# myshell-ai/OpenVoice

Measured on NVIDIA H100. Metric: audio_seconds_per_second, higher is better.
Workload: dtype f32 (3xFP16 split-precision tensor-core convs with fp32 accumulation, fp32 FFMA elsewhere)

## Files before the change

include/ovc.h:

```cpp
#ifndef OVC_B200_H
#define OVC_B200_H

#include <stddef.h>
#include <stdint.h>

#ifdef __cplusplus
extern "C" {
#endif

#define OVC_ABI_VERSION 12

#if defined(__GNUC__)
#define OVC_API __attribute__((visibility("default")))
#else
#define OVC_API
#endif

enum {
  OVC_OK = 0,
  OVC_ERR_INVALID = -1,
  OVC_ERR_CUDA = -2,
  OVC_ERR_STATE = -3,
  OVC_ERR_MISSING = -4,
  OVC_ERR_NOMEM = -5
};

typedef struct ovc_ctx ovc_ctx;

typedef struct ovc_hparams {
  int32_t spec_channels;
  int32_t inter_channels;
  int32_t hidden_channels;
  int32_t gin_channels;
// ... 92 lines not shown

OVC_API int ovc_tts_encode_state(ovc_ctx* ctx, float* stats, int32_t* cum, float* g, void* stream);

OVC_API int ovc_tts_encode_state_rows(ovc_ctx* ctx, const int64_t* dst_row, int N, int Tp, float* stats, int32_t* cum,
                                      float* g, int64_t* y_lengths, void* stream);
OVC_API int ovc_tts_state_rows(ovc_ctx* ctx, const float* stats, const int32_t* cum, const float* g, const int64_t* y_lengths,
                               int B, int T, const int64_t* dst_row, int N, int Tp, float* d_stats, int32_t* d_cum,
                               float* d_g, int64_t* d_y_lengths, void* stream);

OVC_API int ovc_tts_decode_windows(ovc_ctx* ctx, const float* stats, const int32_t* cum, const float* g,
                                   const int64_t* y_lengths, int N, int T, const int64_t* row, const int64_t* frame0,
                                   const int64_t* len, int W, int Wmax, const uint64_t* seed, const int64_t* stream,
                                   const float* noise_scale, float* o, float* z_p, void* cuda_stream);

OVC_API int ovc_set_precision(ovc_ctx* ctx, int mode);

#define OVC_OPT_TTS_SIMPLE 2
#define OVC_OPT_GRAPH 3
#define OVC_OPT_PDL 5
#define OVC_OPT_BRANCHES 7
#define OVC_OPT_PAIR 8
#define OVC_OPT_PAIR_OCC 9
#define OVC_OPT_STAGED_EPI 10
OVC_API int ovc_set_option(ovc_ctx* ctx, int key, int value);

OVC_API int ovc_last_launch_count(const ovc_ctx* ctx);

OVC_API int ovc_graph_replays(const ovc_ctx* ctx);

OVC_API int ovc_profile_enable(ovc_ctx* ctx, int enable);
OVC_API int ovc_profile_read(ovc_ctx* ctx, double* ms, int64_t* launches, double* flops, double* bytes);
OVC_API int ovc_profile_detail(ovc_ctx* ctx, int max, char* names, double* ms, double* flops, double* bytes,
                               int* family);

OVC_API int ovc_debug_enable(ovc_ctx* ctx, int enable);
OVC_API int ovc_debug_fetch(ovc_ctx* ctx, const char* name, float* host_out, size_t max_floats,
                    int64_t* shape4 );

#ifdef __cplusplus
}
#endif
#endif
```

openvoice_b200/_native.py:

```python
from __future__ import annotations

import ctypes as C
import os
from typing import Dict, Iterable, Optional, Tuple

_HERE = os.path.dirname(os.path.abspath(__file__))
LIB_PATH = os.path.join(_HERE, "libovc_b200.so")

ABI_VERSION = 12
EXPORTS = (
    "ovc_abi_version", "ovc_last_error", "ovc_create", "ovc_destroy", "ovc_load_tensor",
    "ovc_finalize_weights", "ovc_workspace_floats", "ovc_voice_conversion", "ovc_last_launch_count",
    "ovc_profile_enable", "ovc_profile_read", "ovc_profile_detail", "ovc_debug_enable", "ovc_debug_fetch",
    "ovc_spectrogram", "ovc_convert_waveform", "ovc_set_precision", "ovc_reference_encoder",
    "ovc_tts_info", "ovc_tts_encode", "ovc_tts_decode", "ovc_set_option", "ovc_graph_replays",
    "ovc_reference_encoder_ragged", "ovc_resample", "ovc_resample_span", "ovc_voice_conversion_items",
    "ovc_convert_waveform_items", "ovc_tts_encode_items", "ovc_tts_decode_items", "ovc_philox_normals",
    "ovc_tts_encode_state", "ovc_tts_decode_windows", "ovc_spectrogram_ring", "ovc_splice",
    "ovc_tts_encode_state_rows", "ovc_tts_state_rows",
)

STREAM_OPEN = 2 ** 63 - 1
SPLICE_PCM16 = 1


class OvcHParams(C.Structure):
    _fields_ = [
        ("spec_channels", C.c_int32), ("inter_channels", C.c_int32), ("hidden_channels", C.c_int32),
        ("gin_channels", C.c_int32), ("resblock", C.c_int32), ("n_resblock_kernels", C.c_int32),
        ("resblock_kernel_sizes", C.c_int32 * 4), ("resblock_dilations", (C.c_int32 * 3) * 4),
        ("n_upsamples", C.c_int32), ("upsample_rates", C.c_int32 * 4),
        ("upsample_kernel_sizes", C.c_int32 * 4), ("upsample_initial_channel", C.c_int32),
# ... 208 lines not shown
        used, ignored = [], []
        for k, v in sd.items():
            a = v.detach().cpu().float().contiguous().numpy() if hasattr(v, "detach") else np.ascontiguousarray(v, dtype=np.float32)
            if a.ndim == 0 or a.ndim > 4:
                ignored.append(k)
                continue
            shape = (C.c_int64 * a.ndim)(*a.shape)
            rc = self.lib.ovc_load_tensor(self.handle, k.encode(), a.ctypes.data_as(C.c_void_p), shape, a.ndim)
            _check(self.lib, rc, f"ovc_load_tensor({k})")
            (ignored if rc == 1 else used).append(k)
        self.finalized = False
        return used, ignored

    def finalize(self):
        _check(self.lib, self.lib.ovc_finalize_weights(self.handle), "ovc_finalize_weights")
        self.finalized = True

    def set_precision(self, mode: str):
        m = PRECISIONS[mode]
        _check(self.lib, self.lib.ovc_set_precision(self.handle, m), "ovc_set_precision")
        self.precision = mode

    def set_option(self, key: str, value: int):
        k = {"tts_simple": 2, "graph": 3, "pdl": 5, "branches": 7, "pair": 8, "pair_occ": 9, "staged_epi": 10}[key]
        _check(self.lib, self.lib.ovc_set_option(self.handle, k, int(value)), "ovc_set_option")

    def voice_conversion(self, spec, lengths, g_src, g_tgt, noise=None, tau: float = 0.3, seed: int = 0,
                         ragged: bool = False, latents: bool = True, stream=None, items: Optional[dict] = None, out=None):
        import torch
        assert spec.is_cuda and spec.dtype == torch.float32 and spec.is_contiguous()
        assert lengths.is_cuda and lengths.dtype == torch.int64 and lengths.is_contiguous()
        B, S, T = spec.shape
        gs = g_src.reshape(B, -1).contiguous().float()
        gt = g_tgt.reshape(B, -1).contiguous().float()
        if noise is not None:
            noise = noise.contiguous().float()
            assert tuple(noise.shape) == (B, self.hp.inter_channels, T)
        hop = self.hp.hop_length
        if out is not None:
            assert out.is_cuda and out.dtype == torch.float32 and out.is_contiguous() and out.numel() == B * hop * T
            o = out.view(B, 1, hop * T)
        else:
            o = torch.empty(B, 1, hop * T, device=spec.device, dtype=torch.float32)
        lat = None
        if latents:
            lat = tuple(torch.empty(B, self.hp.inter_channels, T, device=spec.device, dtype=torch.float32)
                        for _ in range(3))
# ... 332 lines not shown
```

openvoice_b200/csrc/ovc_lib.cu:

```cuda
#include <cuda_runtime.h>

#include <algorithm>
#include <cmath>
#include <cstdarg>
#include <cstdio>
#include <cstdlib>
#include <cstring>
#include <map>
#include <string>
#include <vector>

#include "../../include/ovc.h"
#include "ovc_convpack.h"
#include "ovc_small.cuh"
#include "ovc_tcconv.cuh"
#include "ovc_tts.cuh"
#include "ovc_refenc.cuh"
#include "ovc_resample.cuh"
#include "ovc_splice.h"
#include "ovc_variants.h"

namespace ovc {

static thread_local std::string g_err;
// ... 66 lines not shown
};

struct ConvLayer {
  int variant = -1;
  int rows = 0;
  int row_tiles = 0;
  int cin = 0;
  int n_chunks = 0;
  size_t w_off = 0;
  size_t b_off = 0;
  int K = 1;
  int cout = 0;
  int out_mul = 1;
};

struct TcLayer : TcGeom {
  size_t w_off = 0;
  size_t b_off = 0;
};

struct WNLayers {
  std::vector<ConvLayer> in, rs;
  std::vector<TcLayer> tc_in, tc_rs;
};

struct Fp32Dense { size_t w = 0, b = 0; int Cin = 0, K = 0, N = 0; bool fast = false; ConvLayer cl; };
struct DdsLayers {
  size_t sep_w[3] = {0}, sep_b[3] = {0}, n1g[3] = {0}, n1b[3] = {0}, n2g[3] = {0}, n2b[3] = {0};
  Fp32Dense c1x1[3];
};
struct TtsLayers {
  bool ready = false;
  int n_vocab = 0, n_speakers = 0, H = 0, C = 0, Fc = 0, heads = 0, n_layers = 0, window = 0, D = 0;
  size_t emb = 0, emb_g = 0;
  std::vector<TcLayer> qkv, o;
  std::vector<Fp32Dense> ffn1, ffn2;
  std::vector<size_t> relk, relv, ln1g, ln1b, ln2g, ln2b;
  TcLayer proj;
  Fp32Dense dp_c1, dp_c2, sdp_pre, sdp_proj;
  size_t dp_n1g = 0, dp_n1b = 0, dp_n2g = 0, dp_n2b = 0, dp_pw = 0, dp_pb = 0, dp_cw = 0, dp_cb = 0, sdp_cw = 0, sdp_cb = 0,
         ea = 0;
  DdsLayers dds[4];
  size_t cf_pre_w[4] = {0}, cf_pre_b[4] = {0}, cf_pw[4] = {0}, cf_pb[4] = {0};
};

struct DebugBuf {
// ... 15 lines not shown

  float* d_w = nullptr;
  size_t w_floats = 0;
  std::vector<float> h_w;

  ConvLayer enc_pre, enc_pre16, enc_proj;
  WNLayers enc_wn;
  ConvLayer flow_pre[4], flow_post[4];
  WNLayers flow_wn[4];
  ConvLayer dec_pre, dec_ups[4];
  ConvLayer rb_c1[12][3], rb_c2[12][3];
  TcLayer tc_c1[12][3], tc_c2[12][3], tc_ups[4], tc_pre;
  float* d_tcw = nullptr;
  std::vector<float> h_tcw;
  int precision = 0;
  bool tts_simple = false;
  bool use_graph = true;
  int use_pdl = 2;
  bool use_branches = true;
  int par_frames = 512;
  bool use_pair = true;
  bool use_pair_occ = true;
  bool use_staged_epi = true;
  bool pair_occ2_ok[TCN_N_OCC2] = {};
  cudaStream_t br_stream[2] = {nullptr, nullptr};
  cudaEvent_t br_ev[4] = {nullptr, nullptr, nullptr, nullptr};
  size_t post_w_off = 0;
  size_t cond_w_off = 0, cond_b_off = 0;
  int* d_cond_wrow = nullptr;
  int* d_cond_sel = nullptr;
  int cond_rows_out = 0;
  int cond_off_enc = 0, cond_off_fsrc = 0, cond_off_ftgt = 0, cond_off_dec = 0;
  int cond_off_enc_tc = 0, cond_off_fsrc_tc = 0, cond_off_ftgt_tc = 0;

  float2* d_tw = nullptr;
  float* d_win = nullptr;

  bool has_refenc = false;
  size_t re_conv_w[6] = {0}, re_conv_b[6] = {0}, re_wih = 0, re_whh = 0, re_bih = 0, re_bhh = 0, re_pw = 0, re_pb = 0,
         re_lng = 0, re_lnb = 0;
  int re_gru_in = 0;
  float* d_re = nullptr;
  size_t re_floats = 0;

  std::map<std::pair<int64_t, int64_t>, double*> rs_banks;
  bool rs_smem_opt_in = false;
// ... 177 lines not shown
  const int H = 192;
  *out = WNLayers();
  for (int i = 0; i < n_layers; ++i) {
    HostTensor w, r;
    const HostTensor* rb;
    const std::string prs = prefix + ".res_skip_layers." + std::to_string(i);
    const int rows = (i < n_layers - 1) ? 2 * H : H;
    TRY(conv_weight(c, prefix + ".in_layers." + std::to_string(i), {2 * H, H, 5}, &w));
    TRY(conv_weight(c, prs, {rows, H, 1}, &r));
    TRY(tensor(c, prs + ".bias", {rows}, &rb));
    out->in.push_back(pack_conv(
        c, V_WN_IN, 2 * H, H,
        [&](int p, int ci, int k) { return w.data[((size_t)paired_row(p, H) * H + ci) * 5 + k]; },
        [&](int) { return 0.f; }, 0, 5, 2 * H));
    out->rs.push_back(pack_conv(
        c, V_WN_RS, rows, H, [&](int p, int ci, int) { return r.data[(size_t)p * H + ci]; },
        [&](int p) { return rb->data[p]; }, rows, 1, rows));
    out->tc_in.push_back(pack_tc(
        c, 2 * H, H, 5, 1, [&](int p, int ci, int k) { return w.data[((size_t)paired_row32(p, H) * H + ci) * 5 + k]; },
        [&](int) { return 0.f; }));
    out->tc_rs.push_back(pack_tc(
        c, rows, H, 1, 1, [&](int p, int ci, int) { return r.data[(size_t)p * H + ci]; },
        [&](int p) { return rb->data[p]; }));
  }
  return OVC_OK;
}

#include "ovc_tts_pack.inc"

static int finalize(ovc_ctx* c) {
  const ovc_hparams& hp = c->hp;
  const int H = 192, S = hp.spec_channels, G = hp.gin_channels;
  drop_graphs(c);
  c->h_w.clear();
  c->h_tcw.clear();

  {
    const HostTensor *w, *b, *pw, *pb;
    TRY(tensor(c, "enc_q.pre.weight", {H, S, 1}, &w));
    TRY(tensor(c, "enc_q.pre.bias", {H}, &b));
    c->enc_pre = pack_conv(c, V_ENC_PRE, H, S, [&](int p, int ci, int) { return w->data[(size_t)p * S + ci]; },
                           [&](int p) { return b->data[p]; }, H, 1, H);
    c->enc_pre16 = c->enc_pre;
    c->enc_pre16.variant = V_FLOW_PRE;
    TRY(pack_wn(c, "enc_q.enc", 16, &c->enc_wn));
    TRY(tensor(c, "enc_q.proj.weight", {2 * H, H, 1}, &pw));
// ... 148 lines not shown
      TRY(tensor(c, e.key, e.shape, &t));
      *e.off = append(c->h_w, t->data);
    }
    c->has_refenc = true;
  }
  c->tts = TtsLayers();
  if (find(c, "enc_p.emb.weight")) TRY(pack_tts(c));
  ON_DEVICE(c);
  if (c->d_w) { cudaFree(c->d_w); c->d_w = nullptr; }
  c->w_floats = c->h_w.size();
  CK(cudaMalloc(&c->d_w, c->w_floats * sizeof(float)));
  CK(cudaMemcpy(c->d_w, c->h_w.data(), c->w_floats * sizeof(float), cudaMemcpyHostToDevice));
  if (c->d_tcw) { cudaFree(c->d_tcw); c->d_tcw = nullptr; }
  CK(cudaMalloc(&c->d_tcw, c->h_tcw.size() * sizeof(float)));
  CK(cudaMemcpy(c->d_tcw, c->h_tcw.data(), c->h_tcw.size() * sizeof(float), cudaMemcpyHostToDevice));
  c->h_tcw.clear();
  c->h_tcw.shrink_to_fit();
  for (int TN : {128, 64, 32})
    for (bool staged : {false, true}) {
      const TcKernel k = tc_conv_kernel(TN, staged), p = tc_pair_kernel(TN, TcPairOcc(), staged);
      CK(cudaFuncSetAttribute(k.fn, cudaFuncAttributeMaxDynamicSharedMemorySize, (int)k.smem));
      CK(cudaFuncSetAttribute(p.fn, cudaFuncAttributeMaxDynamicSharedMemorySize, (int)p.smem));
    }
  for (int i = 0; i < TCN_N_OCC2; ++i) {
    const TcKernel k = tc_pair_kernel(kTcPairOcc2[i].C, kTcPairOcc2[i].o);
    CK(cudaFuncSetAttribute(k.fn, cudaFuncAttributeMaxDynamicSharedMemorySize, (int)k.smem));
    int blocks = 0;
    CK(cudaOccupancyMaxActiveBlocksPerMultiprocessor(&blocks, k.fn, k.threads, k.smem));
    c->pair_occ2_ok[i] = blocks >= 2;
    if (blocks < 2)
      fprintf(stderr, "ovc: the C = %d conv-pair kernel with %d operand buffer(s) fits %d CTA(s) per SM, not 2; its pairs run "
              "one CTA per SM\n", kTcPairOcc2[i].C, kTcPairOcc2[i].o.nabuf, blocks);
  }
  if (c->d_cond_wrow) cudaFree(c->d_cond_wrow);
  if (c->d_cond_sel) cudaFree(c->d_cond_sel);
  CK(cudaMalloc(&c->d_cond_wrow, wrow.size() * sizeof(int)));
  CK(cudaMalloc(&c->d_cond_sel, sel.size() * sizeof(int)));
  CK(cudaMemcpy(c->d_cond_wrow, wrow.data(), wrow.size() * sizeof(int), cudaMemcpyHostToDevice));
  CK(cudaMemcpy(c->d_cond_sel, sel.data(), sel.size() * sizeof(int), cudaMemcpyHostToDevice));
  if (!c->d_tw) {
    std::vector<float2> tw(STFT_N);
    std::vector<float> win(STFT_N);
    const double PI = 3.14159265358979323846;
    for (int m = 0; m < STFT_N; ++m) {
      tw[m] = make_float2((float)std::cos(2.0 * PI * m / STFT_N), (float)(-std::sin(2.0 * PI * m / STFT_N)));
      win[m] = (float)(0.5 - 0.5 * std::cos(2.0 * PI * m / STFT_N));
// ... 109 lines not shown
static int prof_begin(Run& r) {
  ovc_ctx* c = r.c;
  if (!c->prof) return OVC_OK;
  if (c->ev_used + 2 > c->ev.size()) {
    const size_t old = c->ev.size();
    c->ev.resize(old + 512);
    for (size_t i = old; i < c->ev.size(); ++i) CK(cudaEventCreate(&c->ev[i]));
  }
  CK(cudaEventRecord(c->ev[c->ev_used], r.st));
  return OVC_OK;
}
static int prof_end(Run& r, int variant, int family, double flops, double bytes, int tag = 0) {
  ovc_ctx* c = r.c;
  if (!c->prof) return OVC_OK;
  CK(cudaEventRecord(c->ev[c->ev_used + 1], r.st));
  c->ev_used += 2;
  c->ev_flops.push_back(flops);
  c->ev_bytes.push_back(bytes);
  c->ev_variant.push_back(variant);
  c->ev_family.push_back(family);
  c->ev_tag.push_back(tag);
  return OVC_OK;
}
enum { V_TCPAIR128 = -14, V_TCPAIR64 = -12, V_TCPAIR32 = -13, V_TC128 = -1, V_TC64 = -2, V_TC32 = -3, V_TRANSPOSE = -4, V_TTS_DENSE = -5, V_TTS_LN = -6, V_TTS_SCORES = -7,
       V_TTS_ATTN = -8, V_TTS_DW = -9, V_TTS_SPLINE = -10, V_TTS_MISC = -11 };
static const char* variant_name(int v) {
  if (v >= 0) return kInfo[v].name;
  switch (v) {
    case V_TCPAIR128: return "PAIR_N128";
    case V_TCPAIR64: return "PAIR_N64";
    case V_TCPAIR32: return "PAIR_N32";
    case V_TC128: return "TC3_N128";
    case V_TC64: return "TC3_N64";
    case V_TC32: return "TC3_N32";
    case V_TTS_DENSE: return "TTS_DENSE32";
    case V_TTS_LN: return "TTS_LAYERNORM";
    case V_TTS_SCORES: return "TTS_SCORES";
    case V_TTS_ATTN: return "TTS_ATTN_OUT";
    case V_TTS_DW: return "TTS_DWCONV";
    case V_TTS_SPLINE: return "TTS_SPLINE";
    case V_TTS_MISC: return "TTS_MISC";
    default: return "TRANSPOSE";
  }
}

struct TcExtra {
  int epi = 0;
  const float* bias = nullptr;
  long long bias_bs = 0;
  float* s = nullptr;
  int split = 0, first = 0;
// ... 98 lines not shown
  const int n = (int)wn.in.size();
  for (int i = 0; i < n; ++i) {
    ConvArgs a{};
    a.x = x; a.x_bs = bs; a.x_pitch = P;
    a.bias = cond + (size_t)i * 384; a.bias_bs = cond_bs;
    a.y = acts; a.y_bs = bs; a.y_pitch = P;
    a.lens_in = r.lens; a.lens_out = r.lens; a.mul_in = 1; a.mul_out = 1;
    a.slope = 1.f;
    TRY(launch(r, wn.in[i], a, T));
    ConvArgs b{};
    b.x = acts; b.x_bs = bs; b.x_pitch = P;
    b.bias = r.c->d_w + wn.rs[i].b_off; b.bias_bs = 0;
    b.y = x; b.y_bs = bs; b.y_pitch = P;
    b.s = skip; b.s_bs = bs; b.s_pitch = P;
    b.lens_in = r.lens; b.lens_out = r.lens; b.mul_in = 1; b.mul_out = 1;
    b.slope = 1.f;
    b.split = (i < n - 1) ? 192 : 0;
    b.flags = (i == 0) ? F_FIRST : 0;
    TRY(launch(r, wn.rs[i], b, T));
  }
  return OVC_OK;
}

static int run_wn_tc(Run& r, const WNLayers& wn, float* x, float* skip, float* acts, float* x_cl, float* skip_cl,
                     const float* cond_tc, int cond_bs) {
  const int P = r.P, T = r.Tmax;
  const int n = (int)wn.tc_in.size();
  TRY(launch_transpose(r, x, x_cl, 192, P));
  for (int i = 0; i < n; ++i) {
    TcExtra g;
    g.epi = 1; g.bias = cond_tc + (size_t)i * 384; g.bias_bs = cond_bs; g.y_ld = 192; g.use_lens_frames = true;
    TRY(launch_tc(r, wn.tc_in[i], x_cl, acts, nullptr, T, 1, 1.f, 1.f, 0, 0, g));
    TcExtra q;
    q.epi = 2; q.s = skip_cl; q.split = (i < n - 1) ? 192 : 0; q.first = (i == 0); q.y_ld = 192; q.use_lens_frames = true;
    TRY(launch_tc(r, wn.tc_rs[i], acts, x_cl, nullptr, T, 1, 1.f, 1.f, 0, 0, q));
  }
  TRY(launch_transpose(r, skip_cl, skip, P, 192));
  return OVC_OK;
}

static int run_flow(Run& r, const WsLayout& W, float* ws, bool reverse, const float* cond_all) {
  ovc_ctx* c = r.c;
  const int P = r.P, T = r.Tmax;
  const long long bs = 192LL * P;
  float* z = ws + W.z;
  float* x = ws + W.x;
  float* skip = ws + W.skip;
  float* acts = ws + W.acts;
  const int sect = reverse ? c->cond_off_ftgt : c->cond_off_fsrc;
  for (int step = 0; step < 4; ++step) {
    const int f = reverse ? 3 - step : step;
// ... 89 lines not shown
  }
  const cudaError_t ie = cudaGraphInstantiate(&e->exec, graph, 0);
  cudaGraphDestroy(graph);
  if (ie != cudaSuccess) {
    cudaGetLastError();
    e->exec = nullptr;
    e->seen = -1000000;
    return body(st);
  }
  e->launches = c->launches;
  CK(cudaGraphLaunch(e->exec, st));
  c->graph_replays++;
  return OVC_OK;
}

static int set_call_params(ovc_ctx* c, uint64_t seed, float tau, const ItemParams& items, cudaStream_t st) {
  if (!c->d_callp) CK(cudaMalloc(&c->d_callp, sizeof(CallParams)));
  set_call_params_kernel<<<1, 1, 0, st>>>(c->d_callp, seed, tau, items);
  CK(cudaGetLastError());
  return OVC_OK;
}
static uintptr_t option_bits(const ovc_ctx* c) {
  return (uintptr_t)c->precision | ((uintptr_t)c->use_pdl << 15) | ((uintptr_t)c->use_branches << 14) | ((uintptr_t)c->use_pair << 17) |
         ((uintptr_t)c->use_pair_occ << 18) | ((uintptr_t)c->use_staged_epi << 19);
}

static int ensure_ws(ovc_ctx* c, const WsLayout& W, int B, int Tmax, cudaStream_t st) {
  if (W.total <= c->ws_floats) return OVC_OK;
  CK(cudaStreamSynchronize(st));
  drop_graphs(c);
  if (c->d_ws) CK(cudaFree(c->d_ws));
  c->d_ws = nullptr;
  c->ws_floats = 0;
  cudaError_t e = cudaMalloc(&c->d_ws, W.total * sizeof(float));
  if (e != cudaSuccess) {
    cudaGetLastError();
    return fail(OVC_ERR_NOMEM, "workspace of %.2f GB for B=%d Tmax=%d does not fit: %s", W.total * 4e-9, B, Tmax,
                cudaGetErrorString(e));
  }
  c->ws_floats = W.total;
  return OVC_OK;
}

static int copy_latent_out(Run& r, const WsLayout& W, float* ws, float* dst) {
  if (!dst) return OVC_OK;
  dim3 grid((r.Tmax + 255) / 256, 192, r.B);
  copy_latent_kernel<<<grid, 256, 0, r.st>>>(ws + W.z, W.P, dst, r.Tmax, 192, r.lens);
// ... 728 lines not shown
  return OVC_OK;
}

int ovc_set_precision(ovc_ctx* c, int mode) {
  if (!c) return fail(OVC_ERR_INVALID, "null context");
  if (mode < 0 || mode > 2) return fail(OVC_ERR_INVALID, "precision mode must be 0 (fp32 FFMA), 1 (3xFP16 tensor cores) or 2 (single-pass fp16)");
  c->precision = mode;
  return OVC_OK;
}

int ovc_set_option(ovc_ctx* c, int key, int value) {
  if (!c) return fail(OVC_ERR_INVALID, "null context");
  switch (key) {
    case OVC_OPT_TTS_SIMPLE: c->tts_simple = value != 0; return OVC_OK;
    case OVC_OPT_GRAPH: c->use_graph = value != 0; return OVC_OK;
    case OVC_OPT_PDL:
      if (value < 0 || value > 2) return fail(OVC_ERR_INVALID, "pdl must be 0, 1 or 2");
      c->use_pdl = value;
      return OVC_OK;
    case OVC_OPT_BRANCHES: c->use_branches = value != 0; return OVC_OK;
    case OVC_OPT_PAIR: c->use_pair = value != 0; return OVC_OK;
    case OVC_OPT_PAIR_OCC: c->use_pair_occ = value != 0; return OVC_OK;
    case OVC_OPT_STAGED_EPI: c->use_staged_epi = value != 0; return OVC_OK;
    default: return fail(OVC_ERR_INVALID, "unknown option %d", key);
  }
}

int ovc_last_launch_count(const ovc_ctx* c) { return c ? c->launches : 0; }

int ovc_graph_replays(const ovc_ctx* c) { return c ? c->graph_replays : 0; }

int ovc_profile_enable(ovc_ctx* c, int enable) {
  if (!c) return fail(OVC_ERR_INVALID, "null context");
  c->prof = enable != 0;
  c->ev_used = 0;
  c->ev_flops.clear();
  c->ev_bytes.clear();
  c->ev_variant.clear();
  c->ev_family.clear();
  c->ev_tag.clear();
  return OVC_OK;
}

int ovc_profile_read(ovc_ctx* c, double* ms, int64_t* launches, double* flops, double* bytes) {
  if (!c) return fail(OVC_ERR_INVALID, "null context");
  double tms = 0, tf = 0, tb = 0;
// ... 9 lines not shown
  }
  if (ms) *ms = tms;
  if (launches) *launches = n;
  if (flops) *flops = tf;
  if (bytes) *bytes = tb;
  c->ev_used = 0;
  c->ev_flops.clear();
  c->ev_bytes.clear();
  c->ev_variant.clear();
  c->ev_family.clear();
  c->ev_tag.clear();
  return OVC_OK;
}

int ovc_profile_detail(ovc_ctx* c, int max, char* names , double* ms, double* flops, double* bytes, int* family) {
  if (!c) return fail(OVC_ERR_INVALID, "null context");
  int n = 0;
  for (size_t i = 0; i + 1 < c->ev_used && n < max; i += 2, ++n) {
    float m = 0;
    CK(cudaEventElapsedTime(&m, c->ev[i], c->ev[i + 1]));
    if (names) {
      const int tag = c->ev_tag[i / 2], v = c->ev_variant[i / 2];
      if (tag && v == V_TCPAIR128) snprintf(names + 16 * n, 16, "T128Pk%dd%d", (tag >> 8) & 255, tag & 255);
      else if (tag && (v == V_TCPAIR64 || v == V_TCPAIR32)) snprintf(names + 16 * n, 16, "P%dk%dd%d", tag >> 16, (tag >> 8) & 255, tag & 255);
      else if (tag) snprintf(names + 16 * n, 16, "T%dc%dk%dd%d", v == V_TC128 ? 128 : v == V_TC64 ? 64 : 32, tag >> 16, (tag >> 8) & 255, tag & 255);
      else { strncpy(names + 16 * n, variant_name(v), 15); names[16 * n + 15] = 0; }
    }
    if (ms) ms[n] = m;
    if (flops) flops[n] = c->ev_flops[i / 2];
    if (bytes) bytes[n] = c->ev_bytes[i / 2];
    if (family) family[n] = c->ev_family[i / 2];
  }
  return n;
}

int ovc_debug_enable(ovc_ctx* c, int enable) {
  if (!c) return fail(OVC_ERR_INVALID, "null context");
  c->debug = enable != 0;
  return OVC_OK;
}

int ovc_debug_fetch(ovc_ctx* c, const char* name, float* host_out, size_t max_floats, int64_t* shape4) {
  if (!c || !name) return fail(OVC_ERR_INVALID, "null argument");
  auto it = c->taps.find(name);
  if (it == c->taps.end()) return fail(OVC_ERR_INVALID, "no debug tap named '%s' (enable debug and run a call first)", name);
  const DebugBuf& d = it->second;
// ... 13 lines not shown
```

openvoice_b200/csrc/ovc_tcconv.cuh:

```cuda
#pragma once
#include "ovc_conv.cuh"
#include "ovc_tc.cuh"
#include "ovc_tcpack.h"

namespace ovc {

struct TcConvArgs {
  const float* x; long long x_bs;
  const uint16_t* w;
  const float* bias; long long bias_bs;
  float* y; long long y_bs; int y_ld;
  const float* r;
  float* s; long long s_bs;
  int epi;
  int split; int first;
  const long long* lens; int tmax; int mul;
  const long long* lens_x; int has_lens_x;
  int Cin; int Ntot; int K; int DIL;
  float slope; float scale; int accumulate;
  int passes;
  const uint16_t* w2; const float* bias2;
};

__device__ __forceinline__ void pdl_launch_dependents() { asm volatile("griddepcontrol.launch_dependents;" ::: "memory"); }
// ... 92 lines not shown
__device__ __forceinline__ void tc_epilogue(const TcConvArgs& a, const float (&d)[TN], int b, int t0, int n0, int lim, int row_a) {
  const bool two = a.passes == 3;
  tc_epilogue_v<TN>(a, [&](int j) { return tc_result<TN>(d, two, j); }, b, t0, n0, lim, row_a);
}
__device__ __forceinline__ TcConvArgs tc_pair_epilogue_args(const TcConvArgs& a, int TN) {
  TcConvArgs e = a;
  e.y_ld = TN; e.r = a.x; e.bias = a.bias2; e.bias_bs = 0; e.epi = 0;
  return e;
}

template <int TN>
__device__ __forceinline__ void tc_mma_step(float (&d)[TN], uint64_t a_hi, uint64_t a_lo, uint64_t b, bool three, bool first) {
  float (&lo)[TN / 2] = *reinterpret_cast<float(*)[TN / 2]>(&d[TN / 2]);
  float (&hi)[TN / 2] = *reinterpret_cast<float(*)[TN / 2]>(&d[0]);
  tc::Wgmma<TN>::mma(hi, a_hi, b, first ? 0 : 1);
  if (three) {
    tc::Wgmma<TN>::mma(lo, a_hi, b + TN, first ? 0 : 1);
    tc::Wgmma<TN>::mma(lo, a_lo, b, 1);
  }
}

constexpr int TCN_THREADS = 384;
constexpr int TCN_NCT = 96;

template <int TN, bool PAIR, int OCC = 1, int NAB = 2, bool STAGED = false>
struct TcnCfg {
  static_assert(!PAIR || TN == 32 || TN == 64 || TN == 128, "conv pairs: C = 32, 64 or 128");
  static_assert(OCC == 1 || (PAIR && TN <= 64), "two CTAs per SM: C = 32 / 64 pairs");
  static_assert(!STAGED || (TN == 128 && OCC == 1), "staged epilogue: TN = 128, one CTA per SM");
  static constexpr int THREADS = STAGED ? TCN_THREADS + 128 : TCN_THREADS;
  static constexpr int KCH = 32, NKC = KCH / 8;
  static constexpr int ROWS = 194;
  static constexpr int ROWS2 = TCN_ROWS2;
  static constexpr int NABUF = NAB;
  static constexpr int RING = PAIR ? tc_pair_ring(TN, OCC, NAB) : tc_ring_slots(TN, PAIR);
  static constexpr int SLOT_BYTES = 2 * 2 * TN * 16;
  static constexpr int A_BUF_BYTES = 2 * NKC * ROWS * 16;
  static constexpr int A2_BYTES = PAIR ? 2 * (TN / 8) * ROWS2 * 16 : 0;
  static constexpr int STAGE_BYTES = STAGED ? (TN / 2) * 256 * 4 : 0;
  static_assert(!STAGED || !PAIR || STAGE_BYTES <= A2_BYTES, "a pair's staging tile lies in its conv-2 operand");
  static constexpr int SBUF_BYTES = STAGED && !PAIR ? STAGE_BYTES : 0;
  static constexpr size_t SMEM_BYTES = 1024 + NABUF * A_BUF_BYTES + A2_BYTES + RING * SLOT_BYTES + SBUF_BYTES;
  static_assert(!PAIR || SMEM_BYTES == tc_pair_smem(TN, NABUF, RING), "tc_pair_smem");
  static_assert(SMEM_BYTES <= (OCC == 1 ? 232448 : TCN_SMEM_OCC2), "shared memory budget");
  static_assert((2 * NABUF + 2 * RING + 2) * 8 <= 1024, "barrier area");
  static constexpr int PROD_REGS = OCC == 1 && !STAGED ? 56 : 32, MMA_REGS = STAGED ? 184 : OCC == 1 ? 224 : 104;
// ... 287 lines not shown
}
inline bool tc_stage_pays(int K, int passes) { return passes * K >= 15; }
inline TcKernel tc_conv_kernel(int TN, bool staged) {
  if (TN == 128) return staged ? tc_kernel<128, false, 1, 2, true>() : tc_kernel<128, false>();
  if (TN == 64) return tc_kernel<64, false>();
  if (TN == 32) return tc_kernel<32, false>();
  return {};
}
inline TcKernel tc_pair_kernel(int C, TcPairOcc o, bool staged = false) {
  if (o.occ == 1 && o.nabuf == 2) {
    if (C == 128) return staged ? tc_kernel<128, true, 1, 2, true>() : tc_kernel<128, true>();
    if (C == 64) return tc_kernel<64, true>();
    if (C == 32) return tc_kernel<32, true>();
  } else if (o.occ == 2) {
    if (C == 32 && o.nabuf == 2) return tc_kernel<32, true, 2, 2>();
    if (C == 32 && o.nabuf == 1) return tc_kernel<32, true, 2, 1>();
    if (C == 64 && o.nabuf == 1) return tc_kernel<64, true, 2, 1>();
  }
  return {};
}
constexpr int TCN_N_OCC2 = 3;
constexpr struct { int C; TcPairOcc o; } kTcPairOcc2[TCN_N_OCC2] = {{32, {2, 2}}, {32, {2, 1}}, {64, {2, 1}}};

template <int C>
__global__ void __launch_bounds__(256) conv_post_cl_kernel(const float* __restrict__ x, long long x_bs,
                                                           const float* __restrict__ w, float* __restrict__ y,
                                                           long long y_bs, int y_len, const long long* lens, int tmax,
                                                           int mul) {
  constexpr int TB = 256, ROWS = TB + 6, LD = ROWS + 3;
  __shared__ float ws[7][C];
  __shared__ float xs[C][LD];
  for (int i = threadIdx.x; i < C * 7; i += blockDim.x) ws[i % 7][i / 7] = w[i];
  const int b = blockIdx.y;
  const int lim = (lens ? (int)min((long long)tmax, lens[b]) : tmax) * mul;
  const int t0 = blockIdx.x * TB;
  const float* xb = x + (size_t)b * x_bs;
  for (int idx = threadIdx.x; idx < ROWS * (C / 4); idx += blockDim.x) {
    const int row = idx / (C / 4), q = idx % (C / 4);
    const int tt = t0 - 3 + row;
    float4 v = make_float4(0.f, 0.f, 0.f, 0.f);
    if (tt >= 0 && tt < lim) v = *reinterpret_cast<const float4*>(xb + (size_t)tt * C + 4 * q);
    xs[4 * q + 0][row] = v.x > 0.f ? v.x : 0.01f * v.x;
    xs[4 * q + 1][row] = v.y > 0.f ? v.y : 0.01f * v.y;
    xs[4 * q + 2][row] = v.z > 0.f ? v.z : 0.01f * v.z;
    xs[4 * q + 3][row] = v.w > 0.f ? v.w : 0.01f * v.w;
  }
// ... 34 lines not shown
```

openvoice_b200/csrc/ovc_tcpack.h:

```cpp
#pragma once
#include <cuda_fp16.h>
#include <stddef.h>
#include <stdint.h>

#include <algorithm>

namespace ovc {

constexpr int TCN_HMAX = 25;
constexpr int TCN_ROWS2 = 146;

constexpr int tc_ring_slots(int TN, bool pair) {
  return pair ? (TN == 32 ? 44 : TN == 64 ? 24 : 12) : (TN == 32 ? 22 : 12);
}

struct TcGeom {
  int Cin = 0, Ntot = 0, K = 0, DIL = 1, TN = 0;
};

inline int tc_tile_n(int Ntot, int Cin, int K, int DIL) {
  if (Ntot <= 0 || Cin <= 0 || K <= 0 || DIL <= 0) return 0;
  if (Ntot % 32 || Cin % 32 || (K - 1) / 2 * DIL > TCN_HMAX) return 0;
  return Ntot % 128 == 0 ? 128 : (Ntot % 64 == 0 ? 64 : 32);
}
// ... 33 lines not shown
}

template <class RAW>
inline float tc_ups_weight(RAW raw, int s, int kk, int cout, int row, int ci, int tap) {
  const int pad = (kk - s) / 2;
  const int ph = row / cout, co = row % cout;
  const int kidx = s * (1 - tap) + ph + pad;
  return (kidx >= 0 && kidx < kk) ? raw(ci, co, kidx) : 0.f;
}

inline bool tc_pair_fits(const TcGeom& T1, const TcGeom& T2) {
  if (!(T1.TN == 32 || T1.TN == 64)) return false;
  const int ring = tc_ring_slots(T1.TN, true);
  return T1.Ntot == T1.TN && T1.Cin == T1.TN && T2.Ntot == T1.TN && T2.Cin == T1.TN && T2.TN == T1.TN && T2.K == T1.K &&
         T2.DIL == 1 && (T1.K - 1) / 2 * T1.DIL <= TCN_HMAX && 2 * (T1.Cin / 16) * T1.K <= ring && T1.K <= 5;
}

inline bool tc_pair_fuses(const TcGeom& T1, const TcGeom& T2) {
  if (!(T1.TN == 32 || T1.TN == 64 || T1.TN == 128)) return false;
  return T1.Ntot == T1.TN && T1.Cin == T1.TN && T2.Ntot == T1.TN && T2.Cin == T1.TN && T2.TN == T1.TN && T2.K == T1.K &&
         T2.DIL == 1 && (T1.K - 1) / 2 * T1.DIL <= TCN_HMAX && 128 + 2 * ((T2.K - 1) / 2) <= TCN_ROWS2;
}

struct TcGrid {
  int n_tt = 0, total = 0, grid_x = 0, ncol = 0;
};
inline TcGrid tc_grid(int t_len, int B, int Ntot, int TN, int sm_count, int grid_div) {
  TcGrid g;
  g.n_tt = (t_len + 127) / 128;
  g.total = g.n_tt * B;
  g.ncol = Ntot / TN;
  const int per_col = std::max(1, sm_count / g.ncol / std::max(1, grid_div));
  g.grid_x = std::min(g.total, per_col);
  return g;
}
inline TcGrid tc_pair_grid(int t_len, int B, int K, int sm_count, int occ = 1) {
  TcGrid g;
  const int R = 128 - (K - 1);
  g.n_tt = (t_len + R - 1) / R;
  g.total = g.n_tt * B;
  g.ncol = 1;
  g.grid_x = std::min(g.total, occ * sm_count);
  return g;
}

constexpr size_t tc_pair_smem(int TN, int nabuf, int ring) {
  return 1024 + (size_t)nabuf * 2 * 4 * 194 * 16 + (size_t)2 * (TN / 8) * TCN_ROWS2 * 16 + (size_t)ring * 2 * 2 * TN * 16;
}
constexpr size_t TCN_SMEM_OCC2 = (233472 - 2 * 1024) / 2;
constexpr int tc_pair_ring(int TN, int occ, int nabuf) {
  return occ == 1 ? tc_ring_slots(TN, true) : (int)((TCN_SMEM_OCC2 - tc_pair_smem(TN, nabuf, 0)) / (2 * 2 * TN * 16));
}

struct TcPairOcc {
  int occ = 1, nabuf = 2;
};
// ... 12 lines not shown
```

Measured before the change: 2411.

## Fuse WaveNet in-conv, gated activation and res/skip conv into one kernel

```diff
diff --git a/include/ovc.h b/include/ovc.h
--- a/include/ovc.h
+++ b/include/ovc.h
@@ -8,7 +8,7 @@
 extern "C" {
 #endif
 
-#define OVC_ABI_VERSION 12
+#define OVC_ABI_VERSION 13
 
 #if defined(__GNUC__)
 #define OVC_API __attribute__((visibility("default")))
@@ -147,6 +147,7 @@
 #define OVC_OPT_PAIR 8
 #define OVC_OPT_PAIR_OCC 9
 #define OVC_OPT_STAGED_EPI 10
+#define OVC_OPT_WN_FUSE 11
 OVC_API int ovc_set_option(ovc_ctx* ctx, int key, int value);
 
 OVC_API int ovc_last_launch_count(const ovc_ctx* ctx);
diff --git a/openvoice_b200/_native.py b/openvoice_b200/_native.py
--- a/openvoice_b200/_native.py
+++ b/openvoice_b200/_native.py
@@ -7,7 +7,7 @@
 _HERE = os.path.dirname(os.path.abspath(__file__))
 LIB_PATH = os.path.join(_HERE, "libovc_b200.so")
 
-ABI_VERSION = 12
+ABI_VERSION = 13
 EXPORTS = (
     "ovc_abi_version", "ovc_last_error", "ovc_create", "ovc_destroy", "ovc_load_tensor",
     "ovc_finalize_weights", "ovc_workspace_floats", "ovc_voice_conversion", "ovc_last_launch_count",
@@ -262,7 +262,8 @@
         self.precision = mode
 
     def set_option(self, key: str, value: int):
-        k = {"tts_simple": 2, "graph": 3, "pdl": 5, "branches": 7, "pair": 8, "pair_occ": 9, "staged_epi": 10}[key]
+        k = {"tts_simple": 2, "graph": 3, "pdl": 5, "branches": 7, "pair": 8, "pair_occ": 9, "staged_epi": 10,
+             "wn_fuse": 11}[key]
         _check(self.lib, self.lib.ovc_set_option(self.handle, k, int(value)), "ovc_set_option")
 
     def voice_conversion(self, spec, lengths, g_src, g_tgt, noise=None, tau: float = 0.3, seed: int = 0,
diff --git a/openvoice_b200/csrc/ovc_lib.cu b/openvoice_b200/csrc/ovc_lib.cu
--- a/openvoice_b200/csrc/ovc_lib.cu
+++ b/openvoice_b200/csrc/ovc_lib.cu
@@ -112,6 +112,7 @@
 struct WNLayers {
   std::vector<ConvLayer> in, rs;
   std::vector<TcLayer> tc_in, tc_rs;
+  std::vector<TcLayer> tc_rsf;
 };
 
 struct Fp32Dense { size_t w = 0, b = 0; int Cin = 0, K = 0, N = 0; bool fast = false; ConvLayer cl; };
@@ -173,6 +174,7 @@
   bool use_pair = true;
   bool use_pair_occ = true;
   bool use_staged_epi = true;
+  bool use_wn_fuse = true;
   bool pair_occ2_ok[TCN_N_OCC2] = {};
   cudaStream_t br_stream[2] = {nullptr, nullptr};
   cudaEvent_t br_ev[4] = {nullptr, nullptr, nullptr, nullptr};
@@ -396,6 +398,14 @@
     out->tc_rs.push_back(pack_tc(
         c, rows, H, 1, 1, [&](int p, int ci, int) { return r.data[(size_t)p * H + ci]; },
         [&](int p) { return rb->data[p]; }));
+    const int rows_f = tc_wn_rs_rows_packed(rows);
+    if (rows_f == rows) {
+      out->tc_rsf.push_back(out->tc_rs.back());
+    } else {
+      out->tc_rsf.push_back(pack_tc(
+          c, rows_f, H, 1, 1, [&](int p, int ci, int) { return p < rows ? r.data[(size_t)p * H + ci] : 0.f; },
+          [&](int p) { return p < rows ? rb->data[p] : 0.f; }));
+    }
   }
   return OVC_OK;
 }
@@ -590,6 +600,7 @@
       CK(cudaFuncSetAttribute(k.fn, cudaFuncAttributeMaxDynamicSharedMemorySize, (int)k.smem));
       CK(cudaFuncSetAttribute(p.fn, cudaFuncAttributeMaxDynamicSharedMemorySize, (int)p.smem));
     }
+  CK(cudaFuncSetAttribute(tcwn_kernel, cudaFuncAttributeMaxDynamicSharedMemorySize, (int)TcWnCfg::SMEM_BYTES));
   for (int i = 0; i < TCN_N_OCC2; ++i) {
     const TcKernel k = tc_pair_kernel(kTcPairOcc2[i].C, kTcPairOcc2[i].o);
     CK(cudaFuncSetAttribute(k.fn, cudaFuncAttributeMaxDynamicSharedMemorySize, (int)k.smem));
@@ -745,11 +756,12 @@
   c->ev_tag.push_back(tag);
   return OVC_OK;
 }
-enum { V_TCPAIR128 = -14, V_TCPAIR64 = -12, V_TCPAIR32 = -13, V_TC128 = -1, V_TC64 = -2, V_TC32 = -3, V_TRANSPOSE = -4, V_TTS_DENSE = -5, V_TTS_LN = -6, V_TTS_SCORES = -7,
+enum { V_TCWN = -15, V_TCPAIR128 = -14, V_TCPAIR64 = -12, V_TCPAIR32 = -13, V_TC128 = -1, V_TC64 = -2, V_TC32 = -3, V_TRANSPOSE = -4, V_TTS_DENSE = -5, V_TTS_LN = -6, V_TTS_SCORES = -7,
        V_TTS_ATTN = -8, V_TTS_DW = -9, V_TTS_SPLINE = -10, V_TTS_MISC = -11 };
 static const char* variant_name(int v) {
   if (v >= 0) return kInfo[v].name;
   switch (v) {
+    case V_TCWN: return "WN_FUSED";
     case V_TCPAIR128: return "PAIR_N128";
     case V_TCPAIR64: return "PAIR_N64";
     case V_TCPAIR32: return "PAIR_N32";
@@ -894,11 +906,49 @@
   return OVC_OK;
 }
 
+static int launch_wn_layer(Run& r, const TcLayer& Tin, const TcLayer& Trs, const float* x_in, float* x_out, float* skip,
+                           const float* cond, int cond_bs, int split, int first) {
+  TcWnArgs w{};
+  TcConvArgs& a = w.g;
+  a.x = x_in; a.x_bs = 192LL * r.P;
+  a.w = reinterpret_cast<const uint16_t*>(r.c->d_tcw + Tin.w_off);
+  a.bias = cond; a.bias_bs = cond_bs;
+  a.w2 = reinterpret_cast<const uint16_t*>(r.c->d_tcw + Trs.w_off); a.bias2 = r.c->d_tcw + Trs.b_off;
+  a.lens = r.lens; a.tmax = r.Tmax; a.mul = 1;
+  a.Cin = Tin.Cin; a.Ntot = Tin.Ntot; a.K = Tin.K; a.DIL = Tin.DIL;
+  a.slope = 1.f; a.scale = 1.f;
+  a.passes = r.c->precision == 2 ? 1 : 3;
+  w.x_out = x_out; w.s = skip; w.split = split; w.first = first; w.rs_n = split + 192;
+  const TcGrid g = tc_wn_grid(r.Tmax, r.B, r.c->sm_count);
+  TRY(prof_begin(r));
+  CK(launch_ex(tcwn_kernel, dim3((unsigned)g.grid_x, 1, 1), TCN_THREADS, TcWnCfg::SMEM_BYTES, r.st, r.c->use_pdl != 0, w,
+               g.n_tt, g.total));
+  CK(cudaGetLastError());
+  r.c->launches++;
+  const double units = (double)r.B * r.Tmax;
+  TRY(prof_end(r, V_TCWN, 0, 2.0 * 192 * (384.0 * Tin.K + w.rs_n) * units, 4.0 * 192 * (2 + 2 + (first ? 0 : 1)) * units,
+               (Tin.Cin << 16) | (Tin.K << 8) | Tin.DIL));
+  return OVC_OK;
+}
+
 static int run_wn_tc(Run& r, const WNLayers& wn, float* x, float* skip, float* acts, float* x_cl, float* skip_cl,
                      const float* cond_tc, int cond_bs) {
   const int P = r.P, T = r.Tmax;
   const int n = (int)wn.tc_in.size();
   TRY(launch_transpose(r, x, x_cl, 192, P));
+  bool fuse = r.c->use_wn_fuse;
+  for (int i = 0; i < n; ++i) fuse = fuse && tc_wn_fuses(wn.tc_in[i], wn.tc_rs[i], r.c->precision == 2 ? 1 : 3);
+  if (fuse) {
+    float* xa = x_cl;
+    float* xb = acts;
+    for (int i = 0; i < n; ++i) {
+      TRY(launch_wn_layer(r, wn.tc_in[i], wn.tc_rsf[i], xa, xb, skip_cl, cond_tc + (size_t)i * 384, cond_bs,
+                          (i < n - 1) ? 192 : 0, i == 0));
+      std::swap(xa, xb);
+    }
+    TRY(launch_transpose(r, skip_cl, skip, P, 192));
+    return OVC_OK;
+  }
   for (int i = 0; i < n; ++i) {
     TcExtra g;
     g.epi = 1; g.bias = cond_tc + (size_t)i * 384; g.bias_bs = cond_bs; g.y_ld = 192; g.use_lens_frames = true;
@@ -1034,7 +1084,8 @@
 }
 static uintptr_t option_bits(const ovc_ctx* c) {
   return (uintptr_t)c->precision | ((uintptr_t)c->use_pdl << 15) | ((uintptr_t)c->use_branches << 14) | ((uintptr_t)c->use_pair << 17) |
-         ((uintptr_t)c->use_pair_occ << 18) | ((uintptr_t)c->use_staged_epi << 19);
+         ((uintptr_t)c->use_pair_occ << 18) | ((uintptr_t)c->use_staged_epi << 19) |
+         ((uintptr_t)c->use_wn_fuse << 20);
 }
 
 static int ensure_ws(ovc_ctx* c, const WsLayout& W, int B, int Tmax, cudaStream_t st) {
@@ -1809,6 +1860,7 @@
     case OVC_OPT_PAIR: c->use_pair = value != 0; return OVC_OK;
     case OVC_OPT_PAIR_OCC: c->use_pair_occ = value != 0; return OVC_OK;
     case OVC_OPT_STAGED_EPI: c->use_staged_epi = value != 0; return OVC_OK;
+    case OVC_OPT_WN_FUSE: c->use_wn_fuse = value != 0; return OVC_OK;
     default: return fail(OVC_ERR_INVALID, "unknown option %d", key);
   }
 }
@@ -1864,6 +1916,7 @@
     if (names) {
       const int tag = c->ev_tag[i / 2], v = c->ev_variant[i / 2];
       if (tag && v == V_TCPAIR128) snprintf(names + 16 * n, 16, "T128Pk%dd%d", (tag >> 8) & 255, tag & 255);
+      else if (tag && v == V_TCWN) snprintf(names + 16 * n, 16, "WNFc%dk%d", tag >> 16, (tag >> 8) & 255);
       else if (tag && (v == V_TCPAIR64 || v == V_TCPAIR32)) snprintf(names + 16 * n, 16, "P%dk%dd%d", tag >> 16, (tag >> 8) & 255, tag & 255);
       else if (tag) snprintf(names + 16 * n, 16, "T%dc%dk%dd%d", v == V_TC128 ? 128 : v == V_TC64 ? 64 : 32, tag >> 16, (tag >> 8) & 255, tag & 255);
       else { strncpy(names + 16 * n, variant_name(v), 15); names[16 * n + 15] = 0; }
diff --git a/openvoice_b200/csrc/ovc_tcconv.cuh b/openvoice_b200/csrc/ovc_tcconv.cuh
--- a/openvoice_b200/csrc/ovc_tcconv.cuh
+++ b/openvoice_b200/csrc/ovc_tcconv.cuh
@@ -138,6 +138,39 @@
 
 constexpr int TCN_THREADS = 384;
 constexpr int TCN_NCT = 96;
+
+template <int ROWS, int NKC, int PB>
+__device__ __forceinline__ void tc_convert_chunk(const float* xb, int Cin, int c0, int r0, int items, int lim_x, float slope,
+                                                 unsigned char* ah, int pt) {
+  unsigned char* al = ah + NKC * ROWS * 16;
+  for (int i0 = pt; i0 < items; i0 += TCN_NCT * PB) {
+    float4 v0[PB], v1[PB];
+#pragma unroll
+    for (int u = 0; u < PB; ++u) {
+      const int i = i0 + TCN_NCT * u;
+      const int row = i >> 2, kc = i & 3;
+      const int t = r0 + row;
+      v0[u] = make_float4(0.f, 0.f, 0.f, 0.f);
+      v1[u] = v0[u];
+      if (i < items && t >= 0 && t < lim_x) {
+        const float4* src = reinterpret_cast<const float4*>(xb + (size_t)t * Cin + c0 + kc * 8);
+        v0[u] = src[0];
+        v1[u] = src[1];
+      }
+    }
+#pragma unroll
+    for (int u = 0; u < PB; ++u) {
+      const int i = i0 + TCN_NCT * u;
+      if (i >= items) break;
+      const int row = i >> 2, kc = i & 3;
+      uint4 hi, lo;
+      tc::split_f16x8(v0[u], v1[u], slope, hi, lo);
+      *reinterpret_cast<uint4*>(ah + (kc * ROWS + row) * 16) = hi;
+      *reinterpret_cast<uint4*>(al + (kc * ROWS + row) * 16) = lo;
+    }
+  }
+  asm volatile("fence.proxy.async.shared::cta;" ::: "memory");
+}
 
 template <int TN, bool PAIR, int OCC = 1, int NAB = 2, bool STAGED = false>
 struct TcnCfg {
@@ -471,6 +504,256 @@
 constexpr int TCN_N_OCC2 = 3;
 constexpr struct { int C; TcPairOcc o; } kTcPairOcc2[TCN_N_OCC2] = {{32, {2, 2}}, {32, {2, 1}}, {64, {2, 1}}};
 
+struct TcWnArgs {
+  TcConvArgs g;
+  float* x_out;
+  float* s;
+  int split, first;
+  int rs_n;
+};
+
+struct TcWnCfg {
+  static constexpr int H = 192, GROUNDS = 2 * H / 128;
+  static constexpr int KCH = 32, NKC = KCH / 8, ROWS = 194;
+  static constexpr int NABUF = 2, RING = 10;
+  static constexpr int SLOT_BYTES = 2 * 2 * 128 * 16;
+  static constexpr int A_BUF_BYTES = 2 * NKC * ROWS * 16;
+  static constexpr int ACT_ROWS = 128, ACT_BYTES = 2 * (H / 8) * ACT_ROWS * 16;
+  static constexpr size_t SMEM_BYTES = 1024 + NABUF * A_BUF_BYTES + ACT_BYTES + RING * SLOT_BYTES;
+  static_assert(A_BUF_BYTES == 24832 && ACT_BYTES == 98304 && SMEM_BYTES == 230912, "shared memory layout");
+  static_assert(SMEM_BYTES <= 232448, "shared memory budget");
+  static_assert((2 * NABUF + 2 * RING) * 8 <= 1024, "barrier area");
+  static constexpr int PB = 6;
+  static constexpr int PROD_REGS = 88, MMA_REGS = 208;
+  static constexpr int CTA_REGS = TCN_THREADS * 168;
+  static_assert(128 * PROD_REGS + 256 * MMA_REGS <= CTA_REGS, "register budget");
+  static_assert(TCN_NCT * PB >= (128 + 2 * 2 + 7) / 8 * 8 * NKC, "a k = 5 chunk in one pass");
+};
+
+__device__ __forceinline__ void tc_wn_gate_epilogue(const TcConvArgs& a, const float (&d)[128], bool two, int b, int t0, int n0,
+                                                    int lim, int row_a, unsigned char* act) {
+  constexpr int LBO = TcWnCfg::ACT_ROWS * 16, LO = (TcWnCfg::H / 8) * LBO;
+  const int csub = (threadIdx.x & 3) * 2;
+  const float* bias = a.bias + (size_t)b * a.bias_bs;
+  const int ta = t0 + row_a, tb = ta + 8;
+  const bool oka = ta < lim, okb = tb < lim;
+#pragma unroll
+  for (int c0 = 0; c0 < 128; c0 += 32) {
+    float v[16];
+#pragma unroll
+    for (int i = 0; i < 16; ++i) v[i] = tc_result<128>(d, two, c0 / 2 + i);
+#pragma unroll
+    for (int g = 0; g < 4; ++g) {
+      const float2 bq = __ldg(reinterpret_cast<const float2*>(bias + n0 + c0 + 8 * g + csub));
+      v[4 * g] += bq.x; v[4 * g + 1] += bq.y; v[4 * g + 2] += bq.x; v[4 * g + 3] += bq.y;
+    }
+#pragma unroll
+    for (int g = 0; g < 2; ++g) {
+      float x[4];
+#pragma unroll
+      for (int i = 0; i < 4; ++i) x[i] = tanhf(v[4 * g + i]) * sigmoidf_acc(v[4 * (g + 2) + i]);
+      if (!oka) x[0] = x[1] = 0.f;
+      if (!okb) x[2] = x[3] = 0.f;
+      const __half2 ha = __floats2half2_rn(x[0], x[1]), hb = __floats2half2_rn(x[2], x[3]);
+      const float2 fa = __half22float2(ha), fb = __half22float2(hb);
+      const __half2 la = __floats2half2_rn((x[0] - fa.x) * tc::kLoScale, (x[1] - fa.y) * tc::kLoScale);
+      const __half2 lb = __floats2half2_rn((x[2] - fb.x) * tc::kLoScale, (x[3] - fb.y) * tc::kLoScale);
+      const int cb = (n0 + c0) / 16 + g;
+      const int oa = cb * LBO + row_a * 16 + csub * 2, ob = oa + 8 * 16;
+      *reinterpret_cast<__half2*>(act + oa) = ha;
+      *reinterpret_cast<__half2*>(act + ob) = hb;
+      *reinterpret_cast<__half2*>(act + LO + oa) = la;
+      *reinterpret_cast<__half2*>(act + LO + ob) = lb;
+    }
+  }
+}
+
+template <int NC>
+__device__ __forceinline__ void tc_wn_rs_epilogue(const TcWnArgs& w, const float (&d)[128], bool two, int b, int t0, int n0,
+                                                  int lim, int row_a) {
+  constexpr int LD = TcWnCfg::H;
+  const int csub = (threadIdx.x & 3) * 2;
+  const size_t bo = (size_t)b * w.g.x_bs;
+  const int ta = t0 + row_a, tb = ta + 8;
+  const bool oka = ta < lim, okb = tb < lim;
+#pragma unroll
+  for (int c0 = 0; c0 < NC; c0 += 32) {
+    float v[16];
+#pragma unroll
+    for (int i = 0; i < 16; ++i) v[i] = tc_result<128>(d, two, c0 / 2 + i);
+#pragma unroll
+    for (int g = 0; g < 4; ++g) {
+      const float2 bq = __ldg(reinterpret_cast<const float2*>(w.g.bias2 + n0 + c0 + 8 * g + csub));
+      v[4 * g] += bq.x; v[4 * g + 1] += bq.y; v[4 * g + 2] += bq.x; v[4 * g + 3] += bq.y;
+    }
+    const int col = n0 + c0;
+    const bool to_x = col < w.split;
+    const bool add = to_x || !w.first;
+    const float* src = (to_x ? w.g.x + bo + col : w.s + bo + (col - w.split)) + csub;
+    float* dst = (to_x ? w.x_out + bo + col : w.s + bo + (col - w.split)) + csub;
+    float2 qa[4], qb[4];
+#pragma unroll
+    for (int g = 0; g < 4; ++g) {
+      qa[g] = add && oka ? *reinterpret_cast<const float2*>(src + (size_t)ta * LD + 8 * g) : make_float2(0.f, 0.f);
+      qb[g] = add && okb ? *reinterpret_cast<const float2*>(src + (size_t)tb * LD + 8 * g) : make_float2(0.f, 0.f);
+    }
+#pragma unroll
+    for (int g = 0; g < 4; ++g) {
+      float2 oa = make_float2(v[4 * g], v[4 * g + 1]), ob = make_float2(v[4 * g + 2], v[4 * g + 3]);
+      if (add) {
+        oa = make_float2(qa[g].x + oa.x, qa[g].y + oa.y);
+        ob = make_float2(qb[g].x + ob.x, qb[g].y + ob.y);
+      }
+      if (oka) *reinterpret_cast<float2*>(dst + (size_t)ta * LD + 8 * g) = oa;
+      if (okb) *reinterpret_cast<float2*>(dst + (size_t)tb * LD + 8 * g) = ob;
+    }
+  }
+}
+
+__global__ void __launch_bounds__(TCN_THREADS, 1) tcwn_kernel(const TcWnArgs w, int n_tt, int total) {
+  using Cfg = TcWnCfg;
+  constexpr int ROWS = Cfg::ROWS, NABUF = Cfg::NABUF, RING = Cfg::RING, NKC = Cfg::NKC, GR = Cfg::GROUNDS;
+  const TcConvArgs& a = w.g;
+  extern __shared__ __align__(128) unsigned char smem_raw[];
+  uint64_t* bars = reinterpret_cast<uint64_t*>(smem_raw);
+  uint64_t *a_full = bars, *a_empty = bars + NABUF, *b_full = a_empty + NABUF, *b_empty = b_full + RING;
+  unsigned char* abuf = smem_raw + 1024;
+  unsigned char* act = abuf + NABUF * Cfg::A_BUF_BYTES;
+  unsigned char* bring = act + Cfg::ACT_BYTES;
+
+  const int tid = threadIdx.x, lane = tid & 31;
+  const int warp = __shfl_sync(0xffffffffu, tid >> 5, 0);
+  const int H1 = (a.K - 1) / 2 * a.DIL;
+  const int rows8 = (128 + 2 * H1 + 7) & ~7;
+  const int nq = a.Cin / Cfg::KCH;
+  const int n_gate = (a.Cin / 16) * a.K;
+  const int n_rs = a.Cin / 16;
+  const int rs_rounds = (w.rs_n + 127) / 128;
+  const int n_w = GR * n_gate + rs_rounds * n_rs;
+  if (H1 > TCN_HMAX || a.Cin != Cfg::H || a.Ntot != 2 * Cfg::H || (w.rs_n != 2 * Cfg::H && w.rs_n != Cfg::H)) __trap();
+  constexpr uint32_t BYTES = Cfg::SLOT_BYTES;
+
+  if (tid == 0) {
+    for (int i = 0; i < NABUF; ++i) { mbar_init(&a_full[i], TCN_NCT); mbar_init(&a_empty[i], 2); }
+    for (int i = 0; i < RING; ++i) { mbar_init(&b_full[i], 1); mbar_init(&b_empty[i], 2); }
+    fence_mbar_init();
+  }
+  __syncthreads();
+  pdl_launch_dependents();
+  if (warp != 0) pdl_wait();
+
+#define TCWN_FOR_TILES                                                                                  \
+  for (int tile = blockIdx.x; tile < total; tile += gridDim.x) {                                        \
+    const int b = tile / n_tt, t0 = (tile % n_tt) * 128;                                                \
+    const int lim = (a.lens ? (int)min((long long)a.tmax, a.lens[b]) : a.tmax) * a.mul;                 \
+    if (t0 >= lim) continue;
+
+  if (warp < 4) {
+    tc::regs_dealloc<Cfg::PROD_REGS>();
+    if (warp == 0) {
+      if (lane == 0) {
+        const unsigned char* wg = reinterpret_cast<const unsigned char*>(a.w);
+        const unsigned char* wr = reinterpret_cast<const unsigned char*>(a.w2);
+        int slot = 0;
+        uint32_t phase = 1;
+        TCWN_FOR_TILES
+          (void)b;
+          for (int it = 0; it < n_w; ++it) {
+            const unsigned char* src = it < GR * n_gate ? wg + (size_t)it * BYTES : wr + (size_t)(it - GR * n_gate) * BYTES;
+            mbar_wait(&b_empty[slot], phase);
+            mbar_expect_tx(&b_full[slot], BYTES);
+            tma_bulk_g2s(bring + slot * BYTES, src, BYTES, &b_full[slot]);
+            if (++slot == RING) { slot = 0; phase ^= 1; }
+          }
+        }
+      }
+    } else {
+      const int pt = tid - 32;
+      int buf = 0;
+      uint32_t ephase = 1;
+      TCWN_FOR_TILES
+        const float* xb = a.x + (size_t)b * a.x_bs;
+        for (int r = 0; r < GR; ++r)
+          for (int q = 0; q < nq; ++q) {
+            mbar_wait(&a_empty[buf], ephase);
+            tc_convert_chunk<ROWS, NKC, Cfg::PB>(xb, a.Cin, q * Cfg::KCH, t0 - H1, rows8 * NKC, lim, a.slope, abuf + buf * Cfg::A_BUF_BYTES, pt);
+            mbar_arrive(&a_full[buf]);
+            if (++buf == NABUF) { buf = 0; ephase ^= 1; }
+          }
+      }
+    }
+  } else {
+    tc::regs_alloc<Cfg::MMA_REGS>();
+    const int wg = (warp >> 2) - 1;
+    const bool leader = (tid & 127) == 0;
+    const int row_a = 64 * wg + 16 * (warp & 3) + (lane >> 2);
+    constexpr uint32_t LBO_A = ROWS * 16, LBO_ACT = Cfg::ACT_ROWS * 16, LBO_B = 2 * 128 * 16, SBO = 128;
+    constexpr uint32_t A_LO16 = (NKC * ROWS * 16) >> 4, ACT_LO16 = ((Cfg::H / 8) * LBO_ACT) >> 4, SLOT16 = BYTES >> 4;
+    const uint64_t a_proto = tc::make_desc(0, LBO_A, SBO), act_proto = tc::make_desc(0, LBO_ACT, SBO);
+    const uint64_t b_ring = tc::make_desc(0, LBO_B, SBO) + (tc::smem_addr(bring) >> 4);
+    const uint64_t act_desc = act_proto + ((tc::smem_addr(act) + 64 * wg * 16) >> 4);
+    const bool three = a.passes == 3;
+    float d[128];
+#pragma unroll
+    for (int i = 0; i < 128; ++i) d[i] = 0.f;
+    int slot = 0, buf = 0;
+    uint32_t bphase = 0, aphase = 0;
+    const auto step = [&](uint64_t a_hi, uint64_t a_lo, bool first, int& prev) {
+      mbar_wait(&b_full[slot], bphase);
+      tc_mma_step<128>(d, a_hi, a_lo, b_ring + (uint32_t)slot * SLOT16, three, first);
+      tc::wgmma_commit();
+      tc::wgmma_wait<1>();
+      if (leader && prev >= 0) mbar_arrive(&b_empty[prev]);
+      prev = slot;
+      if (++slot == RING) { slot = 0; bphase ^= 1; }
+    };
+    TCWN_FOR_TILES
+      for (int r = 0; r < GR; ++r) {
+        bool first = true;
+        for (int q = 0; q < nq; ++q) {
+          mbar_wait(&a_full[buf], aphase);
+          tc::fence_regs(d);
+          tc::wgmma_fence();
+          int prev = -1;
+          for (int j = 0; j < 2; ++j) {
+            uint64_t a_cur = a_proto + ((tc::smem_addr(abuf + buf * Cfg::A_BUF_BYTES) + 64 * wg * 16 + 2 * j * LBO_A) >> 4);
+            for (int tap = 0; tap < a.K; ++tap) {
+              step(a_cur, a_cur + A_LO16, first, prev);
+              first = false;
+              a_cur += a.DIL;
+            }
+          }
+          tc::wgmma_wait<0>();
+          tc::fence_regs(d);
+          if (leader) {
+            if (prev >= 0) mbar_arrive(&b_empty[prev]);
+            mbar_arrive(&a_empty[buf]);
+          }
+          if (++buf == NABUF) { buf = 0; aphase ^= 1; }
+        }
+        tc_wn_gate_epilogue(a, d, three, b, t0, 128 * r, lim, row_a, act);
+      }
+      asm volatile("fence.proxy.async.shared::cta;" ::: "memory");
+      named_bar_sync(1 + wg, 128);
+      for (int r = 0; r < rs_rounds; ++r) {
+        tc::fence_regs(d);
+        tc::wgmma_fence();
+        int prev = -1;
+        for (int kk = 0; kk < n_rs; ++kk) {
+          const uint64_t a_cur = act_desc + 2 * kk * (LBO_ACT >> 4);
+          step(a_cur, a_cur + ACT_LO16, kk == 0, prev);
+        }
+        tc::wgmma_wait<0>();
+        tc::fence_regs(d);
+        if (leader && prev >= 0) mbar_arrive(&b_empty[prev]);
+        if (w.rs_n - 128 * r >= 128) tc_wn_rs_epilogue<128>(w, d, three, b, t0, 128 * r, lim, row_a);
+        else tc_wn_rs_epilogue<64>(w, d, three, b, t0, 128 * r, lim, row_a);
+      }
+    }
+  }
+#undef TCWN_FOR_TILES
+}
+
 template <int C>
 __global__ void __launch_bounds__(256) conv_post_cl_kernel(const float* __restrict__ x, long long x_bs,
                                                            const float* __restrict__ w, float* __restrict__ y,
diff --git a/openvoice_b200/csrc/ovc_tcpack.h b/openvoice_b200/csrc/ovc_tcpack.h
--- a/openvoice_b200/csrc/ovc_tcpack.h
+++ b/openvoice_b200/csrc/ovc_tcpack.h
@@ -79,6 +79,12 @@
          T2.DIL == 1 && (T1.K - 1) / 2 * T1.DIL <= TCN_HMAX && 128 + 2 * ((T2.K - 1) / 2) <= TCN_ROWS2;
 }
 
+inline bool tc_wn_fuses(const TcGeom& in, const TcGeom& rs, int passes) {
+  return (passes == 3 || passes == 1) && in.Cin == 192 && in.Ntot == 384 && in.K == 5 && in.DIL == 1 && in.TN == 128 &&
+         rs.Cin == 192 && rs.K == 1 && (rs.Ntot == 384 || rs.Ntot == 192) && rs.TN != 0;
+}
+inline int tc_wn_rs_rows_packed(int rs_n) { return (rs_n + 127) / 128 * 128; }
+
 struct TcGrid {
   int n_tt = 0, total = 0, grid_x = 0, ncol = 0;
 };
@@ -89,6 +95,14 @@
   g.ncol = Ntot / TN;
   const int per_col = std::max(1, sm_count / g.ncol / std::max(1, grid_div));
   g.grid_x = std::min(g.total, per_col);
+  return g;
+}
+inline TcGrid tc_wn_grid(int t_len, int B, int sm_count) {
+  TcGrid g;
+  g.n_tt = (t_len + 127) / 128;
+  g.total = g.n_tt * B;
+  g.ncol = 1;
+  g.grid_x = std::min(g.total, sm_count);
   return g;
 }
 inline TcGrid tc_pair_grid(int t_len, int B, int K, int sm_count, int occ = 1) {
```

New measurement: 2475 (median of 6 runs). 2.6% higher.
